# Mrhonor/Mul-Datasets-Semantic-Segmentation

Measured on NVIDIA B200. Metric: labelled pixels/sec (head+OHEM fwd+bwd, mIoU hist), higher is better.
Workload: dtype f32

## Files before the change

mul-datasets-semantic-segmentation_b200/csrc/mds_bwd.cu:

```cuda
#include "tma_util.cuh"

namespace mdseg {
namespace {

using namespace tma;

constexpr int kKC = 8;
constexpr int kBoxW = 36;
constexpr int kStages = 2;
constexpr int kStageFloats = kKC * 2 * kBoxW;
constexpr int kStageBytes = kStageFloats * 4;
constexpr int kCG = 16;
constexpr int kOwn28 = 28;
constexpr int kOwn = kOwn28;
constexpr int kStgW28 = 160;
constexpr int kMaxR = 5;
constexpr int kEnt = 384;
constexpr uint32_t kNoEnt = 0xffffffffu;
#ifndef MDSEG_BWD_BCAST_PIPE
#define MDSEG_BWD_BCAST_PIPE 1
#endif
#ifndef MDSEG_BWD_XP_NOLD
#define MDSEG_BWD_XP_NOLD 0
#endif
#ifndef MDSEG_BWD_XP_NOUSE
#define MDSEG_BWD_XP_NOUSE 0
#endif
#ifndef MDSEG_BWD_XP_NO5
#define MDSEG_BWD_XP_NO5 0
#endif
#ifndef MDSEG_BWD_CHUNK_LEAN
#define MDSEG_BWD_CHUNK_LEAN 1
#endif

template <bool ROW>
struct Lay {
  static constexpr int kOwn = ROW ? 32 : kOwn28;
  static constexpr int kStgW = ROW ? 176 : kStgW28;
  static constexpr size_t kOffCarry = (size_t)kStages * kStageBytes;
  static constexpr size_t kOffLw = kOffCarry + (size_t)kCG * 32 * 4;
  static constexpr size_t kOffLab = kOffLw + (size_t)kMaxR * kStgW * 4;
  static constexpr size_t kOffEnt = kOffLab + (size_t)kMaxR * kStgW;
  static constexpr size_t kOffTile = kOffEnt + (size_t)kEnt * 4;
  static constexpr size_t kOffEptr = kOffTile + (size_t)kKC * kOwn * 4;
  static constexpr size_t kOffBars = kOffEptr + 16;
  static constexpr size_t kOffXbar = kOffBars + (kStages + 1) * 8;
  static constexpr size_t kOffXchg = kOffXbar + 4 * 8;
  static constexpr size_t kOffC5 = (kOffXchg + 2 * kKC * 2 * 4 + 15) / 16 * 16;
  static constexpr size_t kSmem = ROW ? ((kOffC5 + (size_t)kStages * kKC * 8 + 127) / 128) * 128 : kOffXbar;
  static_assert(kCG / kKC + 1 <= 4, "eptr holds one quad offset per chunk of a class group, plus the end");
  static_assert(kOffLw % 16 == 0 && kOffLab % 16 == 0 && kOffEnt % 16 == 0 && kOffTile % 16 == 0 && kOffBars % 8 == 0 &&
                    kOffC5 % 16 == 0,
                "shared memory carve-up alignment");
};
static_assert(Lay<false>::kSmem <= 13568, "16 resident one-warp CTAs per SM need <= 13568 bytes of shared memory each");
static_assert(16 * Lay<true>::kSmem <= 232448, "a 16-warp row CTA must fit the 227 KB of one SM");
constexpr size_t kSmem = Lay<false>::kSmem;
constexpr int kMaxRowWarps = 16;

struct GraphDev {
  const int* csr_ptr;
  const int* csr_col;
  const float* csr_val;
  const int* csc_ptr;
  const int* csr4_ptr;
  const int* csr4_col;
};

struct Args {
  mdseg_src_table src;
  const int32_t* dataset_ids;
  const void* labels;
  Geom gm;
  int ignore;
  const float* loss_px;
  const float* lse_px;
  const mdseg_ohem_state* states;
  const float* grad_out;
  float grad_scale;
  void* out_base[MDSEG_MAX_DATASETS];
  long long out_image_stride[MDSEG_MAX_DATASETS];
  int out_channels[MDSEG_MAX_DATASETS];
  GraphDev g[MDSEG_MAX_DATASETS];
  int zero_invalid;
  float* scrA;
  float* scrB;
  uint8_t* sel8;
  unsigned lite_mask;
  unsigned char lite_strip[kMaxRowWarps];
  int n_lite;
  int c5s;
  float2* col5;
  int c_scr;
  int seg_rows, n_seg, n_strips;
};

__device__ __forceinline__ void bulk_g2s(void* dst, const void* src, uint32_t bytes, uint64_t* bar) {
  asm volatile("cp.async.bulk.shared::cluster.global.mbarrier::complete_tx::bytes [%0], [%1], %2, [%3];" ::"r"(
                   smem_u32(dst)),
               "l"(src), "r"(bytes), "r"(smem_u32(bar))
               : "memory");
}

__device__ __forceinline__ void sts2_if(uint32_t on, uint32_t addr, float a, float b) {
  asm volatile("{ .reg .pred q;\n  setp.ne.u32 q, %0, 0;\n  @q st.shared.v2.f32 [%1], {%2, %3}; }"
               :: "r"(on), "r"(addr), "f"(a), "f"(b) : "memory");
}

__device__ __forceinline__ void sub_onehot2(float2& e, uint32_t lab2, uint32_t c2, float nwabs) {
  asm("{ .reg .pred p, q;\n"
      "  setp.eq.f16x2 p|q, %2, %3;\n"
      "  @p add.f32 %0, %0, %4;\n"
      "  @q add.f32 %1, %1, %4; }"
      : "+f"(e.x), "+f"(e.y)
      : "r"(lab2), "r"(c2), "f"(nwabs));
}

template <typename L>
__global__ void __launch_bounds__(256) mds_bwd_prep_kernel(const Args a, int64_t px_per_image) {
  const int b = blockIdx.y;
  const int d = a.dataset_ids ? a.dataset_ids[b] : 0;
  const bool valid_ds = d >= 0 && d < a.src.n_datasets;
  const int C = valid_ds ? a.src.C[d] : 0;
  SelParams sp;
  sp.thresh = 0.f; sp.kth = 0.f; sp.mode = 0; sp.w = 0.f;
  if (valid_ds) {
    const mdseg_ohem_state* st = a.states + (a.src.seg_per_dataset ? d : 0);
    sp.thresh = st->thresh; sp.kth = st->kth; sp.mode = st->mode;
    sp.w = (a.grad_out ? a.grad_out[a.src.seg_per_dataset ? d : 0] : 1.f) * a.grad_scale * st->inv_n_sel;
  }
  const bool any = valid_ds && fabsf(sp.w) > 0.f;
  const L* labels = (const L*)a.labels;
  const bool lab16 = ((uintptr_t)a.labels & 15) == 0;
  const int64_t base = (int64_t)b * px_per_image;
  for (int64_t q = (int64_t)blockIdx.x * blockDim.x + threadIdx.x; q < px_per_image / 16;
       q += (int64_t)gridDim.x * blockDim.x) {
    const int64_t p = base + q * 16;
    float4 ls[4];
#pragma unroll
    for (int v = 0; v < 4; ++v) ls[v] = __ldcs(reinterpret_cast<const float4*>(a.loss_px + p) + v);
    uint32_t lab[16];
    if (sizeof(L) == 1 && lab16) {
      const uint4 lv = *reinterpret_cast<const uint4*>((const uint8_t*)a.labels + p);
      const uint32_t wv[4] = {lv.x, lv.y, lv.z, lv.w};
#pragma unroll
      for (int i = 0; i < 16; ++i) lab[i] = (wv[i >> 2] >> (8 * (i & 3))) & 0xffu;
    } else {
#pragma unroll
      for (int i = 0; i < 16; ++i) lab[i] = (uint32_t)load_label<L>(labels, p + i);
    }
    uint32_t out[4];
#pragma unroll
    for (int v = 0; v < 4; ++v) {
      const float lsv[4] = {ls[v].x, ls[v].y, ls[v].z, ls[v].w};
      uint32_t packed = 0;
#pragma unroll
// ... 52 lines not shown
#pragma unroll
    for (int i = 0; i < 4; ++i) v[i] = *reinterpret_cast<const float4*>(tile + ((e[i] >> 16) & 7u) * OWN + 4 * t);
#pragma unroll
    for (int i = 0; i < 4; ++i)
      if (col_ok && e[i] != kNoEnt) store4(base + (int64_t)((e[i] & 0xffffu) * (uint32_t)hw), v[i]);
  }
  for (; q < q1; ++q) {
    const uint32_t e = ents[4 * q + o];
    if (col_ok && e != kNoEnt) {
      const float4 v = *reinterpret_cast<const float4*>(tile + (e >> 16) * OWN + 4 * t);
      store4(base + (int64_t)((e & 0xffffu) * (uint32_t)hw), v);
    }
  }
#else
#pragma unroll 4
  for (int q = q0; q < q1; ++q) {
    const uint32_t e = ents[4 * q + o];
    if (col_ok && e != kNoEnt) {
      const float4 v = *reinterpret_cast<const float4*>(tile + (e >> 16) * OWN + 4 * t);
      store4(base + (int64_t)((e & 0xffffu) * (uint32_t)hw), v);
    }
  }
#endif
  __syncwarp();
}

template <typename TO>
__device__ __forceinline__ void store_class(const Args& a, const GraphDev& gd, const Unit& un, TO* outb, int cg, int row,
                                            float v) {
  const int w = a.gm.w;
  if (gd.csr_ptr == nullptr) {
    if (un.own) outb[((int64_t)(un.c_beg + cg) * a.gm.h + row) * w + un.x] = from_f32<TO>(v);
    return;
  }
  const int e0 = __ldg(gd.csr_ptr + un.c_beg + cg), e1 = __ldg(gd.csr_ptr + un.c_beg + cg + 1);
  for (int e = e0; e < e1; ++e) {
    const int u = __ldg(gd.csr_col + e);
    const float val = gd.csr_val ? __ldg(gd.csr_val + e) : 1.f;
    if (un.own) outb[((int64_t)u * a.gm.h + row) * w + un.x] = from_f32<TO>(v * val);
  }
}

template <int STGW>
__device__ __forceinline__ void issue_staging(const Args& a, const Unit& un, int Ys, int R, float* lw2s, uint8_t* labs,
                                              uint64_t* sbar) {
  mbar_expect_tx(sbar, (uint32_t)(R * un.wst * 5));
  for (int j = 0; j < R; ++j) {
    const int64_t p = ((int64_t)un.b * a.gm.H + (Ys + j)) * a.gm.W + un.Xa;
    bulk_g2s(lw2s + j * STGW, a.lse_px + p, (uint32_t)(un.wst * 4), sbar);
    bulk_g2s(labs + j * STGW, a.sel8 + p, (uint32_t)un.wst, sbar);
  }
}

template <bool ROW>
__device__ __noinline__ void skip_chunk(int lane, int k, int cc, bool own, float* scr_first, int64_t scr_stride,
                                        float* carry, float* tile, float* xslot) {
  constexpr int kOwn = Lay<ROW>::kOwn;
  for (int c = 0; c < cc; ++c) {
    if (ROW && xslot != nullptr && lane == 31) { xslot[2 * c] = 0.f; xslot[2 * c + 1] = 0.f; }
    float* cq = carry + (k * kKC + c) * 32 + lane;
    const float rowv = *cq;
    *cq = 0.f;
    if (scr_first != nullptr) {
      if (own) scr_first[c * scr_stride] = 0.f;
    } else if (ROW) {
      tile[c * kOwn + lane] = rowv;
    } else if (lane >= 1 && lane <= kOwn) {
      tile[c * kOwn + lane - 1] = rowv;
    }
  }
}

template <typename TO, int RT, bool NX5, bool ROW>
__device__ __forceinline__ void cell_row(const Args& a, const CUtensorMap* map, const GraphDev& gd, const Unit& un,
                                         TO* outb, int g, int R, int Ys_next, int R_next, const float (&l1w)[5],
                                         const float (&l1h)[kMaxR],
                                         float* stages, uint64_t* bars, float* carry, float* lw2s,
                                         uint8_t* labs, const uint32_t* ents, const int* eptr, float* tile,
                                         float* xmine, uint64_t* xbar_mine, const float* xleft, uint64_t* xbar_left,
                                         bool lite, const float2* c5sm) {
  constexpr int kOwn = Lay<ROW>::kOwn, kStgW = Lay<ROW>::kStgW;
  const int lane = un.lane;
  const float kInf = __int_as_float(0x7f800000);
  float2 LW[RT][2];
  float lw4[RT];
  uint32_t LH[RT][2], lh4[RT];
  uint32_t anysel = 0;
#pragma unroll
  for (int j = 0; j < RT; ++j) {
    float t[5];
    uint32_t hv[5];
#pragma unroll
    for (int i = 0; i < 5; ++i) {
      t[i] = -kInf;
      hv[i] = 255u;
      if (j < R && i < un.nx) {
        hv[i] = labs[j * kStgW + un.sx + i];
        const float off2 = fmaf(-lw2s[j * kStgW + un.sx + i], kLog2e, un.log2w);
        t[i] = hv[i] != 255u ? off2 : -kInf;
      }
      hv[i] = (uint32_t)__half_as_ushort(__ushort2half_rn((unsigned short)hv[i]));
    }
    LW[j][0] = make_float2(t[0], t[1]);
    LW[j][1] = make_float2(t[2], t[3]);
    lw4[j] = t[4];
    LH[j][0] = hv[0] | (hv[1] << 16);
    LH[j][1] = hv[2] | (hv[3] << 16);
    lh4[j] = hv[4] | (0x5bf8u << 16);
    anysel |= (LH[j][0] ^ 0x5bf85bf8u) | (LH[j][1] ^ 0x5bf85bf8u) | (lh4[j] ^ 0x5bf85bf8u);
  }
  __syncwarp();
  if (lane == 0 && g + 1 < un.g1) issue_staging<kStgW>(a, un, Ys_next, R_next, lw2s, labs, &bars[kStages]);
  const bool skip = (ROW || un.cached) && !__any_sync(0xffffffffu, anysel != 0);

  float2 L1H[RT];
#pragma unroll
  for (int j = 0; j < RT; ++j) L1H[j] = dup2(l1h[j]);
  const float2 L1W[2] = {make_float2(l1w[0], l1w[1]), make_float2(l1w[2], l1w[3])};
  const float l1w4 = l1w[4];
  const bool first_partial = (g == un.g0) && (un.g0 > 0);
  TO* orow = outb + (int64_t)g * a.gm.w + un.x0;
  const float nwabs = -fabsf(un.w_signed);
  const float2 K2 = dup2(kLog2e);

#pragma unroll 1
  for (int k = 0; k < un.n_ch; ++k) {
    const int q = (g - un.g0) * un.n_ch + k;
    const int slot = q % kStages;
    const int c_lo = un.c_beg + k * kKC;
    const int cc = (un.c_end - c_lo) < kKC ? (un.c_end - c_lo) : kKC;

    mbar_wait(&bars[slot], (uint32_t)((q / kStages) & 1));
    const int xs = q & 1;
    if (ROW && xmine != nullptr && q >= 2) mbar_wait(&xbar_mine[2 + xs], (uint32_t)(((q >> 1) - 1) & 1));
    const float* Sp = stages + slot * kStageFloats + un.xl;
    if (skip) {
      skip_chunk<ROW>(lane, k, cc, un.own,
                      first_partial ? a.scrA + (((int64_t)un.b * a.n_seg + un.seg) * a.c_scr + c_lo) * a.gm.w + un.x
                                    : nullptr,
                      a.gm.w, carry, tile, xmine ? xmine + xs * kKC * 2 : nullptr);
    } else {
    float n00 = Sp[0], n01 = Sp[1], n10 = Sp[kBoxW], n11 = Sp[kBoxW + 1];
    uint32_t c2 = class_pair(c_lo);
    float* cp = carry + k * kKC * 32 + lane;
    float* tp = tile + (ROW ? lane : lane - 1);
    uint32_t xaddr = 0, xprod = 0;
    if (ROW && xmine != nullptr && lane == 31) { xaddr = smem_u32(xmine + xs * kKC * 2); xprod = 1; }
    asm volatile("" : "+r"(xaddr), "+r"(xprod));
    const float2* x5p = c5sm + slot * kKC;
#pragma unroll 1
    for (int c = 0; c < cc; ++c, c2 = next_class2(c2)) {
      float v00 = n00, v01 = n01, v10 = n10, v11 = n11;
      Sp += 2 * kBoxW;
      if (c + 1 < cc) { n00 = Sp[0]; n01 = Sp[1]; n10 = Sp[kBoxW]; n11 = Sp[kBoxW + 1]; }
      float2 x5 = make_float2(0.f, 0.f);
      if (!NX5 && un.has5 && !MDSEG_BWD_XP_NOLD && !MDSEG_BWD_XP_NOUSE) x5 = x5p[c];
      const float dv0 = v01 - v00, dv1 = v11 - v10;
      const float2 V0 = dup2(v00), DV0 = dup2(dv0), V1 = dup2(v10), DV1 = dup2(dv1);
      float2 CU2, UR2, CL2, LR2;
#pragma unroll
      for (int p = 0; p < 2; ++p) {
        const float2 h0 = fma2(L1W[p], DV0, V0);
        const float2 dd = sub2(fma2(L1W[p], DV1, V1), h0);
        float2 t0, t1;
#pragma unroll
        for (int j = 0; j < RT; ++j) {
          float2 e = ex2_2(fma2(fma2(L1H[j], dd, h0), K2, LW[j][p]));
          sub_onehot2(e, LH[j][p], c2, nwabs);
          t0 = j == 0 ? e : add2(t0, e);
          t1 = j == 0 ? mul2(L1H[j], e) : fma2(L1H[j], e, t1);
        }
        const float2 cu = sub2(t0, t1);
        CU2 = p == 0 ? cu : add2(CU2, cu);
        UR2 = p == 0 ? mul2(L1W[p], cu) : fma2(L1W[p], cu, UR2);
        CL2 = p == 0 ? t1 : add2(CL2, t1);
        LR2 = p == 0 ? mul2(L1W[p], t1) : fma2(L1W[p], t1, LR2);
      }
      float CU = CU2.x + CU2.y, ur = UR2.x + UR2.y, CL = CL2.x + CL2.y, lr = LR2.x + LR2.y;
      if (!NX5 && lite) {
        CU += x5.x; ur = fmaf(l1w4, x5.x, ur);
        CL += x5.y; lr = fmaf(l1w4, x5.y, lr);
      }
      if (NX5) {
        const float h0 = fmaf(l1w4, dv0, v00);
        const float dd = fmaf(l1w4, dv1, v10) - h0;
        float t0 = 0.f, t1 = 0.f;
#pragma unroll
        for (int j = 0; j < RT; ++j) {
          float2 e = make_float2(ex2_approx(fmaf(fmaf(l1h[j], dd, h0), kLog2e, lw4[j])), 0.f);
          sub_onehot2(e, lh4[j], c2, nwabs);
          t0 += e.x;
          t1 = fmaf(l1h[j], e.x, t1);
        }
        const float cu = t0 - t1;
        CU += cu; ur = fmaf(l1w4, cu, ur);
        CL += t1; lr = fmaf(l1w4, t1, lr);
      }
      const float uo = (CU - ur) * un.wsign;
      const float lo = (CL - lr) * un.wsign;
      ur *= un.wsign;
      lr *= un.wsign;
      float gu = __shfl_up_sync(0xffffffffu, ur, 1);
      float gl = __shfl_up_sync(0xffffffffu, lr, 1);
      if (lane == 0) { gu = 0.f; gl = 0.f; }
      if (ROW) {
        sts2_if(xprod, xaddr, ur, lr);
        xaddr += 8;
      }
      const int cg = k * kKC + c;
      const float up = uo + gu;
      const float rowv = up + *cp;
      *cp = lo + gl;
      cp += 32;
      if (first_partial) {
        if (un.own) a.scrA[(((int64_t)un.b * a.n_seg + un.seg) * a.c_scr + (c_lo + c)) * a.gm.w + un.x] = up;
      } else if (ROW || un.cached) {
        if (ROW || (lane >= 1 && lane <= kOwn)) *tp = rowv;
      } else {
        store_class<TO>(a, gd, un, outb, cg, g, rowv);
      }
      tp += kOwn;
    }
    }
    if (ROW) {
      if (xmine != nullptr && lane == 31) mbar_arrive(&xbar_mine[xs]);
      if (xleft != nullptr) {
        mbar_wait(&xbar_left[xs], (uint32_t)((q >> 1) & 1));
        __syncwarp();
        if (lane < cc) {
          const float xu = xleft[(xs * kKC + lane) * 2], xl = xleft[(xs * kKC + lane) * 2 + 1];
          if (first_partial) {
            a.scrA[(((int64_t)un.b * a.n_seg + un.seg) * a.c_scr + (c_lo + lane)) * a.gm.w + un.x0] += xu;
          } else {
            tile[lane * kOwn] += xu;
          }
          carry[(k * kKC + lane) * 32] += xl;
        }
        __syncwarp();
        if (lane == 0) mbar_arrive(&xbar_left[2 + xs]);
      }
    }
    __syncwarp();
    if (lane == 0 && q + kStages < un.n_loads) {
      const int qn = q + kStages;
#if MDSEG_BWD_CHUNK_LEAN
      const int qrow = un.n_ch == 2 ? qn >> 1 : qn, qk = un.n_ch == 2 ? qn & 1 : 0;
#else
      const int qrow = qn / un.n_ch, qk = qn % un.n_ch;
#endif
      mbar_expect_tx(&bars[slot], kStageBytes + (un.c5base ? kKC * 8 : 0));
      load_4d(stages + slot * kStageFloats, map, &bars[slot], un.box_x, un.g0 + qrow, un.c_beg + qk * kKC, un.b);
      if (un.c5base)
        bulk_g2s(const_cast<float2*>(c5sm) + slot * kKC, un.c5base + (un.g0 + qrow) * un.c5row + qk * kKC, kKC * 8,
                 &bars[slot]);
    }
    if (un.cached && !first_partial) broadcast_chunk<TO, kOwn>(un, orow, ents, eptr[k], eptr[k + 1], tile, a.gm.h * a.gm.w);
  }
}

template <typename TO, bool ROW>
__global__ void __launch_bounds__(ROW ? 32 * kMaxRowWarps : 32, ROW ? 1 : 16)
mds_bwd_kernel(const __grid_constant__ Maps maps, const __grid_constant__ Args a) {
  using L = Lay<ROW>;
  constexpr int kOwn = L::kOwn, kStgW = L::kStgW;
  extern __shared__ __align__(128) unsigned char smem_all[];
  const int wi = ROW ? (int)(threadIdx.x >> 5) : 0;
  const int n_w = ROW ? (int)(blockDim.x >> 5) : 1;
  unsigned char* smem_raw = smem_all + (size_t)wi * L::kSmem;
  float* stages = reinterpret_cast<float*>(smem_raw);
  float* carry = reinterpret_cast<float*>(smem_raw + L::kOffCarry);
  float* lw2s = reinterpret_cast<float*>(smem_raw + L::kOffLw);
  uint8_t* labs = smem_raw + L::kOffLab;
  uint32_t* ents = reinterpret_cast<uint32_t*>(smem_raw + L::kOffEnt);
  float* tile = reinterpret_cast<float*>(smem_raw + L::kOffTile);
  int* eptr = reinterpret_cast<int*>(smem_raw + L::kOffEptr);
  uint64_t* bars = reinterpret_cast<uint64_t*>(smem_raw + L::kOffBars);
  float2* c5sm = reinterpret_cast<float2*>(smem_raw + (ROW ? L::kOffC5 : 0));
  const bool has_right = ROW && wi + 1 < n_w, has_left = ROW && wi > 0;
  uint64_t* xbar_mine = has_right ? reinterpret_cast<uint64_t*>(smem_raw + L::kOffXbar) : nullptr;
  float* xmine = has_right ? reinterpret_cast<float*>(smem_raw + L::kOffXchg) : nullptr;
  uint64_t* xbar_left = has_left ? reinterpret_cast<uint64_t*>(smem_raw - L::kSmem + L::kOffXbar) : nullptr;
  const float* xleft = has_left ? reinterpret_cast<const float*>(smem_raw - L::kSmem + L::kOffXchg) : nullptr;

  const Geom& gm = a.gm;
  const int lane = threadIdx.x & 31;
  const int b = blockIdx.z, grp = blockIdx.y;
  const int strip = ROW ? wi : (int)(blockIdx.x % a.n_strips), seg = ROW ? (int)blockIdx.x : (int)(blockIdx.x / a.n_strips);
  const int d = a.dataset_ids ? a.dataset_ids[b] : 0;
  const int h = gm.h, w = gm.w;
  const int x0 = strip * kOwn;
  const int x = ROW ? x0 + lane : x0 + lane - 1;
  const bool own = ROW ? x <= w - 1 : (lane >= 1 && lane <= kOwn && x <= w - 1);
  const int g0 = seg * a.seg_rows;
  const int g1 = (g0 + a.seg_rows < h - 1) ? g0 + a.seg_rows : h - 1;
  const bool last_seg = (g1 == h - 1);

  if (d < 0 || d >= a.src.n_datasets) {
    if (a.zero_invalid && grp == 0) {
      TO* outb = (TO*)a.out_base[0] + (int64_t)b * a.out_image_stride[0];
      for (int u = 0; u < a.out_channels[0]; ++u) zero_rows<TO>(a, outb, u, g0, g1, last_seg, x, own);
    }
    return;
  }
  const int C = a.src.C[d];
  const int c_beg = grp * kCG;
  if (c_beg >= C) return;
  const int c_end = (c_beg + kCG < C) ? c_beg + kCG : C;
  const GraphDev gd = a.g[d];
  TO* outb = (TO*)a.out_base[d] + (int64_t)b * a.out_image_stride[d];
  const mdseg_ohem_state* st = a.states + (a.src.seg_per_dataset ? d : 0);
  const CUtensorMap* map = &maps.m[d];
  const float wsel = (a.grad_out ? a.grad_out[a.src.seg_per_dataset ? d : 0] : 1.f) * a.grad_scale * st->inv_n_sel;

  const bool cell_ok = (x >= 0) && (x <= w - 2) && (ROW || lane <= kOwn);
  int Xbeg = 0, Xend = 0;
  if (cell_ok) cell_span(gm.xm, x, gm.W, Xbeg, Xend);
  const int nx = Xend - Xbeg;
  const unsigned cmask = __ballot_sync(0xffffffffu, cell_ok);
  int Xw0 = 0;
  if (cmask) Xw0 = __shfl_sync(0xffffffffu, Xbeg, __ffs(cmask) - 1);
  float l1w[5];
#pragma unroll
  for (int i = 0; i < 5; ++i) {
    int cell;
    l1w[i] = 0.f;
    if (i < nx) axis_cell(gm.xm, Xbeg + i, cell, l1w[i]);
  }
  const int n5 = __popc(__ballot_sync(0xffffffffu, nx > 4));
  const bool lite = ROW && a.col5 != nullptr && n5 == 1 && ((a.lite_mask >> strip) & 1u);
  const bool nx5 = n5 > 0 && !lite && !MDSEG_BWD_XP_NO5;

  Unit un;
  un.lane = lane; un.b = b; un.seg = seg; un.x = x; un.nx = nx; un.c_beg = c_beg; un.c_end = c_end;
  un.x0 = x0; un.ncols = (w - x0) < kOwn ? (w - x0) : kOwn;
  un.n_ch = (c_end - c_beg + kKC - 1) / kKC;
  un.g0 = g0; un.g1 = g1; un.own = own;
  un.box_x = ROW ? x0 : ((x0 > 0 ? x0 - 1 : 0) & ~3);
  un.xl = cell_ok ? x - un.box_x : 0;
  un.n_loads = (g1 - g0) * un.n_ch;
  un.Xa = Xw0 & ~15;
  un.sx = cell_ok ? Xbeg - un.Xa : 0;
  un.wst = (gm.W - un.Xa) < kStgW ? (gm.W - un.Xa) : kStgW;
  un.w_signed = wsel; un.wsign = wsel < 0.f ? -1.f : 1.f;
  un.log2w = log2f(fabsf(wsel));
  un.cached = false;
  un.has5 = lite && nx > 4 && !MDSEG_BWD_XP_NO5;
  un.c5base = nullptr; un.c5row = 0;
  if (lite && !MDSEG_BWD_XP_NO5 && !MDSEG_BWD_XP_NOLD) {
    un.c5row = (int64_t)(w / 32) * a.c5s;
    un.c5base = a.col5 + ((int64_t)b * (h - 1) * (w / 32) + strip) * a.c5s + c_beg;
  }

  if (lane == 0) {
    prefetch_map(map);
    for (int s = 0; s <= kStages; ++s) mbar_init(&bars[s], 1);
    if (has_right)
      for (int s = 0; s < 4; ++s) mbar_init(&xbar_mine[s], 1);
    mbar_fence_init();
    {
      int Ys0, Ye0;
      cell_span(gm.ym, g0, gm.H, Ys0, Ye0);
      issue_staging<kStgW>(a, un, Ys0, Ye0 - Ys0, lw2s, labs, &bars[kStages]);
    }
    for (int qn = 0; qn < kStages && qn < un.n_loads; ++qn) {
      mbar_expect_tx(&bars[qn], kStageBytes + (un.c5base ? kKC * 8 : 0));
      load_4d(stages + qn * kStageFloats, map, &bars[qn], un.box_x, g0 + qn / un.n_ch, c_beg + (qn % un.n_ch) * kKC,
              b);
      if (un.c5base)
        bulk_g2s(c5sm + qn * kKC, un.c5base + (g0 + qn / un.n_ch) * un.c5row + (qn % un.n_ch) * kKC, kKC * 8, &bars[qn]);
    }
  }
  for (int cg = 0; cg < kCG; ++cg) carry[cg * 32 + lane] = 0.f;
  static_assert(kCG == 2 * kKC, "the channel-list cache is laid out for two chunks per class group");
  if ((gd.csr_ptr == nullptr || gd.csr_val == nullptr) && a.out_channels[d] <= 0xffff &&
      (int64_t)a.out_channels[d] * h * w < 0x7fffffffLL) {
    const int ncls = c_end - c_beg, nc0 = ncls < kKC ? ncls : kKC;
    int myptr = c_beg + lane;
    if (gd.csr_ptr != nullptr) myptr = lane <= ncls ? __ldg(gd.csr_ptr + c_beg + lane) : 0;
    const int p0 = __shfl_sync(0xffffffffu, myptr, 0);
    const int p8 = __shfl_sync(0xffffffffu, myptr, nc0);
    const int pe = __shfl_sync(0xffffffffu, myptr, ncls);
    const int len0 = p8 - p0, len1 = pe - p8;
    const int base1 = (len0 + 3) & ~3;
    const int total = base1 + ((len1 + 3) & ~3);
    if (lane == 0) {
      eptr[0] = 0;
      eptr[1] = base1 >> 2;
      eptr[un.n_ch] = total >> 2;
    }
    for (int eb = 0; eb < pe - p0; eb += 32) {
      const int e = eb + lane;
      int cls = 0;
#pragma unroll
      for (int j = 1; j < kCG; ++j) {
        const int pj = __shfl_sync(0xffffffffu, myptr, j);
        cls += (j < ncls && pj <= p0 + e) ? 1 : 0;
      }
      if (e < pe - p0) {
        const int u = gd.csr_ptr != nullptr ? __ldg(gd.csr_col + p0 + e) : c_beg + e;
        const int pos = cls < kKC ? e : base1 + (e - len0);
        if (pos < kEnt) ents[pos] = (uint32_t)u | ((uint32_t)(cls & (kKC - 1)) << 16);
      }
    }
    if (lane < base1 - len0 && len0 + lane < kEnt) ents[len0 + lane] = kNoEnt;
    if (lane < total - base1 - len1 && base1 + len1 + lane < kEnt) ents[base1 + len1 + lane] = kNoEnt;
    un.cached = total <= kEnt;
  }
  __syncwarp();
  if (ROW) __syncthreads();

  int ys_tab = gm.H;
  if (g0 + lane < h - 1) ys_tab = first_dst_ge(gm.ym, g0 + lane, gm.H);
  for (int g = g0; g < g1; ++g) {
    const int Ys = __shfl_sync(0xffffffffu, ys_tab, g - g0);
    const int Ye = __shfl_sync(0xffffffffu, ys_tab, g - g0 + 1);
    const int R = Ye - Ys;
    float l1h[kMaxR];
#pragma unroll
    for (int j = 0; j < kMaxR; ++j) {
      int cell;
      l1h[j] = 0.f;
      if (j < R) axis_cell(gm.ym, Ys + j, cell, l1h[j]);
    }
    const int Rn = __shfl_sync(0xffffffffu, ys_tab, (g - g0 + 2) & 31) - Ye;
    mbar_wait(&bars[kStages], (uint32_t)((g - g0) & 1));
#define MDSEG_ROW(RT, N5)                                                                                           \
  cell_row<TO, RT, N5, ROW>(a, map, gd, un, outb, g, R, Ye, Rn, l1w, l1h, stages, bars, carry, lw2s, labs, ents, eptr, \
                            tile, xmine, xbar_mine, xleft, xbar_left, lite, c5sm)
    if (R <= 4) {
      if (nx5) MDSEG_ROW(4, true); else MDSEG_ROW(4, false);
    } else {
      if (nx5) MDSEG_ROW(5, true); else MDSEG_ROW(5, false);
    }
#undef MDSEG_ROW
  }

  if (last_seg && un.cached) {
    TO* olast = outb + (int64_t)(h - 1) * w + x0;
    for (int k = 0; k < un.n_ch; ++k) {
      for (int j = 0; j < kKC && k * kKC + j < c_end - c_beg; ++j)
        if (ROW) tile[j * kOwn + lane] = carry[(k * kKC + j) * 32 + lane];
        else if (lane >= 1 && lane <= kOwn) tile[j * kOwn + lane - 1] = carry[(k * kKC + j) * 32 + lane];
      __syncwarp();
      broadcast_chunk<TO, kOwn>(un, olast, ents, eptr[k], eptr[k + 1], tile, h * w);
    }
  } else {
    for (int cg = 0; cg < c_end - c_beg; ++cg) {
      const float v = carry[cg * 32 + lane];
      if (last_seg) {
        store_class<TO>(a, gd, un, outb, cg, h - 1, v);
      } else if (own) {
        a.scrB[(((int64_t)b * a.n_seg + (seg + 1)) * a.c_scr + (c_beg + cg)) * w + x] = v;
      }
    }
  }
  if (grp == 0 && gd.csr_ptr != nullptr && gd.csc_ptr != nullptr) {
    for (int u0 = 0; u0 < a.out_channels[d]; u0 += 32) {
      const int u = u0 + lane;
      const bool empty = u < a.out_channels[d] && __ldg(gd.csc_ptr + u) == __ldg(gd.csc_ptr + u + 1);
      unsigned m = __ballot_sync(0xffffffffu, empty);
      while (m) {
        const int uu = u0 + __ffs(m) - 1;
        m &= m - 1;
        zero_rows<TO>(a, outb, uu, g0, g1, last_seg, x, own);
      }
    }
  }
}

__global__ void __launch_bounds__(32 * kMaxRowWarps) mds_bwd_col5_kernel(const Args a) {
  const Geom& gm = a.gm;
  const int lane = threadIdx.x & 31, strip = a.lite_strip[threadIdx.x >> 5], n_w = a.gm.w / 32;
  const int g = blockIdx.x, b = blockIdx.y;
  const int d = a.dataset_ids ? a.dataset_ids[b] : 0;
  if (d < 0 || d >= a.src.n_datasets) return;
  const int h = gm.h, w = gm.w;
  const int x = strip * 32 + lane;
  int Xbeg = 0, Xend = 0;
  if (x <= w - 2) cell_span(gm.xm, x, gm.W, Xbeg, Xend);
  const unsigned m5 = __ballot_sync(0xffffffffu, Xend - Xbeg > 4);
  if (__popc(m5) != 1) return;
  const int owner = __ffs(m5) - 1;
  const int xo = strip * 32 + owner;
  const int X5 = __shfl_sync(0xffffffffu, Xbeg, owner) + 4;
  int cell;
  float l1w4;
  axis_cell(gm.xm, X5, cell, l1w4);
  int Ys, Ye;
  cell_span(gm.ym, g, gm.H, Ys, Ye);
  const int R = Ye - Ys;
  const int C = a.src.C[d];
  const mdseg_ohem_state* st = a.states + (a.src.seg_per_dataset ? d : 0);
  const float wsel = (a.grad_out ? a.grad_out[a.src.seg_per_dataset ? d : 0] : 1.f) * a.grad_scale * st->inv_n_sel;
  const float log2w = log2f(fabsf(wsel)), nwabs = -fabsf(wsel);
  const float kInf = __int_as_float(0x7f800000);
  float l1h[kMaxR], off[kMaxR];
  int cls[kMaxR];
#pragma unroll
  for (int j = 0; j < kMaxR; ++j) {
    l1h[j] = 0.f; off[j] = -kInf; cls[j] = 255;
    if (j < R) {
      axis_cell(gm.ym, Ys + j, cell, l1h[j]);
      const int64_t p = ((int64_t)b * gm.H + (Ys + j)) * gm.W + X5;
      cls[j] = a.sel8[p];
      if (cls[j] != 255) off[j] = fmaf(-a.lse_px[p], kLog2e, log2w);
    }
  }
  const float* yb = (const float*)a.src.base[d] + (int64_t)b * a.src.image_stride[d] + (int64_t)g * w + xo;
// ... 24 lines not shown
  const int d = a.dataset_ids ? a.dataset_ids[b] : 0;
  if (d < 0 || d >= a.src.n_datasets) return;
  const int C = a.src.C[d];
  const int w = a.gm.w, h = a.gm.h, w4 = w / 4;
  const int idx = blockIdx.x * blockDim.x + threadIdx.x;
  const int cls = idx / w4, x4 = idx - cls * w4;
  if (cls >= C) return;
  const int row = k * a.seg_rows;
  const int64_t so = (((int64_t)b * a.n_seg + k) * a.c_scr + cls) * w + x4 * 4;
  const float4 A = *reinterpret_cast<const float4*>(a.scrA + so);
  const float4 B = *reinterpret_cast<const float4*>(a.scrB + so);
  const float v[4] = {A.x + B.x, A.y + B.y, A.z + B.z, A.w + B.w};
  const GraphDev gd = a.g[d];
  TO* outb = (TO*)a.out_base[d] + (int64_t)b * a.out_image_stride[d];
  if (gd.csr_ptr == nullptr) {
    TO* o = outb + ((int64_t)cls * h + row) * w + x4 * 4;
#pragma unroll
    for (int i = 0; i < 4; ++i) o[i] = from_f32<TO>(v[i]);
    return;
  }
  const int e0 = __ldg(gd.csr_ptr + cls), e1 = __ldg(gd.csr_ptr + cls + 1);
  for (int e = e0; e < e1; ++e) {
    const int u = __ldg(gd.csr_col + e);
    const float val = gd.csr_val ? __ldg(gd.csr_val + e) : 1.f;
    TO* o = outb + ((int64_t)u * h + row) * w + x4 * 4;
#pragma unroll
    for (int i = 0; i < 4; ++i) o[i] = from_f32<TO>(v[i] * val);
  }
}

#ifndef MDSEG_SEG_ROWS
#define MDSEG_SEG_ROWS 16
#endif
int pick_seg_rows(int h, int w, int n_images, int c_max) {
  int sr = h - 1 < MDSEG_SEG_ROWS ? h - 1 : MDSEG_SEG_ROWS;
  if (sr < 1) sr = 1;
  if (!(w % 32 == 0 && w / 32 <= kMaxRowWarps)) return sr;
  const long long per_seg = (long long)n_images * ((c_max + kCG - 1) / kCG);
  while (sr > 4 && per_seg * ((h - 1 + sr - 1) / sr) < sm_count()) sr /= 2;
  return sr;
}

template <typename L>
int launch_prep(const Args& a, int n_images, cudaStream_t s) {
  const int64_t ppi = (int64_t)a.gm.H * a.gm.W;
  int64_t bx = ceil_div64(ppi / 16, 256);
  const int64_t want = ceil_div64((int64_t)sm_count() * 16, n_images);
  if (bx > want) bx = want;
  mds_bwd_prep_kernel<L><<<dim3((unsigned)bx, (unsigned)n_images), 256, 0, s>>>(a, ppi);
  MDSEG_LAUNCH_OK();
  return 0;
}

bool row_route(const Args& a, bool ents_fit) {
  return ents_fit && a.gm.w % 32 == 0 && a.gm.w / 32 <= kMaxRowWarps;
}

template <typename TO>
int launch(int label_dtype, const Maps& maps, const Args& a, int n_images, int max_c, bool ents_fit, cudaStream_t s) {
  int rc = 2;
  switch (label_dtype) {
    case MDSEG_U8: rc = launch_prep<uint8_t>(a, n_images, s); break;
    case MDSEG_I32: rc = launch_prep<int32_t>(a, n_images, s); break;
    case MDSEG_I64: rc = launch_prep<int64_t>(a, n_images, s); break;
    default: set_error("mdseg_mds_bwd: unsupported label dtype %d", label_dtype);
  }
  if (rc) return rc;
  if (row_route(a, ents_fit)) {
    const int n_w = a.gm.w / 32;
    if (a.col5 != nullptr && a.n_lite > 0) {
      mds_bwd_col5_kernel<<<dim3((unsigned)(a.gm.h - 1), (unsigned)n_images), 32 * a.n_lite, 0, s>>>(a);
      MDSEG_LAUNCH_OK();
    }
    const size_t smem = (size_t)n_w * Lay<true>::kSmem;
    auto k = mds_bwd_kernel<TO, true>;
    MDSEG_CUDA_OK(cudaFuncSetAttribute(k, cudaFuncAttributeMaxDynamicSharedMemorySize, (int)smem));
    dim3 grid((unsigned)a.n_seg, (unsigned)((max_c + kCG - 1) / kCG), (unsigned)n_images);
    k<<<grid, 32 * n_w, smem, s>>>(maps, a);
  } else {
    auto k = mds_bwd_kernel<TO, false>;
    MDSEG_CUDA_OK(cudaFuncSetAttribute(k, cudaFuncAttributeMaxDynamicSharedMemorySize, (int)kSmem));
    dim3 grid((unsigned)(a.n_strips * a.n_seg), (unsigned)((max_c + kCG - 1) / kCG), (unsigned)n_images);
    k<<<grid, 32, kSmem, s>>>(maps, a);
  }
  MDSEG_LAUNCH_OK();
  if (a.n_seg > 1) {
    dim3 g2((unsigned)(((int64_t)max_c * (a.gm.w / 4) + 255) / 256), (unsigned)(a.n_seg - 1), (unsigned)n_images);
    mds_bwd_fixup_kernel<TO><<<g2, 256, 0, s>>>(a);
    MDSEG_LAUNCH_OK();
  }
  return 0;
}

size_t col5_bytes(int n_images, int h, int w, int c_max) {
  if (w % 32 != 0 || w / 32 > kMaxRowWarps || h < 2) return 0;
  return (size_t)n_images * (h - 1) * (w / 32) * ((c_max + kKC - 1) / kKC * kKC) * sizeof(float2) + 16;
}

void pick_lite_strips(Args& a) {
  a.lite_mask = 0; a.n_lite = 0;
  if (a.col5 == nullptr) return;
  const int w = a.gm.w, W = a.gm.W;
  int n5[kMaxRowWarps] = {0};
  int cols = 0, cur = 0;
  for (int X = 0; X <= W; ++X) {
    int cell = w - 2;
    if (X < W) {
      const int i0 = (int)(a.gm.xm.scale * (float)X);
      cell = i0 > w - 2 ? w - 2 : i0;
    }
    if (X == W || cell != cur) {
      if (cols > 4 && cur / 32 < kMaxRowWarps) ++n5[cur / 32];
      cur = cell; cols = 0;
    }
    ++cols;
  }
  for (int st = 0; st < w / 32 && st < kMaxRowWarps; ++st)
    if (n5[st] == 1) {
      a.lite_mask |= 1u << st;
      a.lite_strip[a.n_lite++] = (unsigned char)st;
    }
}

int src_max_c(const mdseg_src_table* s) {
  int m = 0;
  for (int i = 0; i < s->n_datasets; ++i) m = s->C[i] > m ? s->C[i] : m;
  return m;
// ... 229 lines not shown
```

Baseline: 11.10 billion.

## Stage full gradient rows in shared memory and write them with bulk async copies

On the row route, each warp now writes its per-chunk gradient tile into a CTA-wide double-buffered row buffer instead of a per-warp tile. The last warp to finish a chunk, found through a shared-memory atomic ticket, broadcasts whole rows to every mapped output channel with cp.async.bulk shared-to-global copies. Mbarriers guard buffer reuse. The aim is to replace many small per-warp scattered global stores with full-row bulk transfers, at the cost of cross-warp synchronisation, serialised issue by a single lane, and a new alignment check on the output.

```diff
diff --git a/mul-datasets-semantic-segmentation_b200/csrc/mds_bwd.cu b/mul-datasets-semantic-segmentation_b200/csrc/mds_bwd.cu
--- a/mul-datasets-semantic-segmentation_b200/csrc/mds_bwd.cu
+++ b/mul-datasets-semantic-segmentation_b200/csrc/mds_bwd.cu
@@ -29,21 +29,28 @@
 #ifndef MDSEG_BWD_XP_NO5
 #define MDSEG_BWD_XP_NO5 0
 #endif
+#ifndef MDSEG_BWD_XP_NOBCAST
+#define MDSEG_BWD_XP_NOBCAST 0
+#endif
 #ifndef MDSEG_BWD_CHUNK_LEAN
 #define MDSEG_BWD_CHUNK_LEAN 1
+#endif
+#ifndef MDSEG_BWD_ROWSTORE
+#define MDSEG_BWD_ROWSTORE 1
 #endif
 
 template <bool ROW>
 struct Lay {
   static constexpr int kOwn = ROW ? 32 : kOwn28;
   static constexpr int kStgW = ROW ? 176 : kStgW28;
+  static constexpr bool kWarpEnts = !(ROW && MDSEG_BWD_ROWSTORE);
   static constexpr size_t kOffCarry = (size_t)kStages * kStageBytes;
   static constexpr size_t kOffLw = kOffCarry + (size_t)kCG * 32 * 4;
   static constexpr size_t kOffLab = kOffLw + (size_t)kMaxR * kStgW * 4;
   static constexpr size_t kOffEnt = kOffLab + (size_t)kMaxR * kStgW;
-  static constexpr size_t kOffTile = kOffEnt + (size_t)kEnt * 4;
-  static constexpr size_t kOffEptr = kOffTile + (size_t)kKC * kOwn * 4;
-  static constexpr size_t kOffBars = kOffEptr + 16;
+  static constexpr size_t kOffTile = kOffEnt + (kWarpEnts ? (size_t)kEnt * 4 : 0);
+  static constexpr size_t kOffEptr = kOffTile + (kWarpEnts ? (size_t)kKC * kOwn * 4 : 0);
+  static constexpr size_t kOffBars = kOffEptr + (kWarpEnts ? 16 : 0);
   static constexpr size_t kOffXbar = kOffBars + (kStages + 1) * 8;
   static constexpr size_t kOffXchg = kOffXbar + 4 * 8;
   static constexpr size_t kOffC5 = (kOffXchg + 2 * kKC * 2 * 4 + 15) / 16 * 16;
@@ -53,10 +60,29 @@
                     kOffC5 % 16 == 0,
                 "shared memory carve-up alignment");
 };
+constexpr int kMaxRowWarps = 16;
+struct RowTail {
+  __host__ __device__ static constexpr size_t kOffEnt(int w) { return (size_t)2 * kKC * w * 4; }
+  __host__ __device__ static constexpr size_t kOffEptr(int w) { return kOffEnt(w) + (size_t)kEnt * 4; }
+  __host__ __device__ static constexpr size_t kOffTicket(int w) { return kOffEptr(w) + 16; }
+  __host__ __device__ static constexpr size_t kOffBars(int w) { return kOffTicket(w) + 2 * 4; }
+  __host__ __device__ static constexpr size_t kBytes(int w) { return kOffBars(w) + 2 * 8; }
+};
+struct RowStore {
+  float* rows;
+  const uint32_t* ents;
+  const int* eptr;
+  unsigned* ticket;
+  uint64_t* empty;
+  int n_w;
+  bool cached;
+};
 static_assert(Lay<false>::kSmem <= 13568, "16 resident one-warp CTAs per SM need <= 13568 bytes of shared memory each");
-static_assert(16 * Lay<true>::kSmem <= 232448, "a 16-warp row CTA must fit the 227 KB of one SM");
+static_assert(kMaxRowWarps * Lay<true>::kSmem + (MDSEG_BWD_ROWSTORE ? RowTail::kBytes(32 * kMaxRowWarps) : 0) <= 232448,
+              "a 16-warp row CTA must fit the 227 KB of one SM");
+static_assert(Lay<true>::kSmem % 16 == 0 && RowTail::kOffBars(32) % 8 == 0, "bulk copies read 16-byte aligned rows");
 constexpr size_t kSmem = Lay<false>::kSmem;
-constexpr int kMaxRowWarps = 16;
+constexpr size_t row_smem(int n_w) { return (size_t)n_w * Lay<true>::kSmem + (MDSEG_BWD_ROWSTORE ? RowTail::kBytes(32 * n_w) : 0); }
 
 struct GraphDev {
   const int* csr_ptr;
@@ -102,6 +128,15 @@
                : "memory");
 }
 
+__device__ __forceinline__ void bulk_s2g(void* dst, const void* src, uint32_t bytes) {
+  asm volatile("cp.async.bulk.global.shared::cta.bulk_group [%0], [%1], %2;" ::"l"(dst), "r"(smem_u32(src)), "r"(bytes)
+               : "memory");
+}
+__device__ __forceinline__ void bulk_commit() { asm volatile("cp.async.bulk.commit_group;" ::: "memory"); }
+__device__ __forceinline__ void bulk_wait_read() { asm volatile("cp.async.bulk.wait_group.read 0;" ::: "memory"); }
+__device__ __forceinline__ void bulk_wait_all() { asm volatile("cp.async.bulk.wait_group 0;" ::: "memory"); }
+__device__ __forceinline__ void fence_async_smem() { asm volatile("fence.proxy.async.shared::cta;" ::: "memory"); }
+
 __device__ __forceinline__ void sts2_if(uint32_t on, uint32_t addr, float a, float b) {
   asm volatile("{ .reg .pred q;\n  setp.ne.u32 q, %0, 0;\n  @q st.shared.v2.f32 [%1], {%2, %3}; }"
                :: "r"(on), "r"(addr), "f"(a), "f"(b) : "memory");
@@ -260,10 +295,63 @@
   }
 }
 
+template <typename TO>
+__device__ __noinline__ void rows_out(const Args& a, const RowStore& rs, TO* outb, int lane, int s, int row, int k,
+                                      int cc) {
+  const int h = a.gm.h, w = a.gm.w;
+  float* buf = rs.rows + s * kKC * w;
+  if (rs.cached) {
+    if constexpr (sizeof(TO) == 2) {
+      __syncwarp();
+      for (int c = 0; c < cc; ++c) {
+        const float2* src = reinterpret_cast<const float2*>(buf + c * w);
+        TO* dst = reinterpret_cast<TO*>(buf) + c * w;
+        float2 v[kMaxRowWarps / 2];
+#pragma unroll
+        for (int i = 0; i < kMaxRowWarps / 2; ++i)
+          if (lane + 32 * i < w / 2) v[i] = src[lane + 32 * i];
+        __syncwarp();
+#pragma unroll
+        for (int i = 0; i < kMaxRowWarps / 2; ++i)
+          if (lane + 32 * i < w / 2) {
+            dst[2 * (lane + 32 * i)] = from_f32<TO>(v[i].x);
+            dst[2 * (lane + 32 * i) + 1] = from_f32<TO>(v[i].y);
+          }
+        __syncwarp();
+      }
+      fence_async_smem();
+      __syncwarp();
+    }
+    if (lane == 0) {
+      const unsigned char* src = reinterpret_cast<const unsigned char*>(buf);
+      const uint32_t bytes = (uint32_t)(w * sizeof(TO));
+      for (int i = 4 * rs.eptr[k]; i < 4 * rs.eptr[k + 1]; ++i) {
+        const uint32_t e = rs.ents[i];
+        if (e != kNoEnt) bulk_s2g(outb + ((int64_t)(e & 0xffffu) * h + row) * w, src + ((e >> 16) & 7u) * bytes, bytes);
+      }
+      bulk_commit();
+      bulk_wait_read();
+    }
+  }
+  if (lane == 0) mbar_arrive(&rs.empty[s]);
+  __syncwarp();
+}
+
+template <typename TO>
+__device__ __forceinline__ void rows_done(const Args& a, const RowStore& rs, TO* outb, int lane, int s, int row, int k,
+                                          int cc) {
+  fence_async_smem();
+  __syncwarp();
+  unsigned t = 0;
+  if (lane == 0)
+    asm volatile("atom.acq_rel.cta.shared::cta.inc.u32 %0, [%1], %2;"
+                 : "=r"(t) : "r"(smem_u32(&rs.ticket[s])), "r"((unsigned)rs.n_w - 1) : "memory");
+  if (__shfl_sync(0xffffffffu, t, 0) == (unsigned)rs.n_w - 1) rows_out<TO>(a, rs, outb, lane, s, row, k, cc);
+}
+
 template <bool ROW>
 __device__ __noinline__ void skip_chunk(int lane, int k, int cc, bool own, float* scr_first, int64_t scr_stride,
-                                        float* carry, float* tile, float* xslot) {
-  constexpr int kOwn = Lay<ROW>::kOwn;
+                                        float* carry, float* tile, int ts, float* xslot) {
   for (int c = 0; c < cc; ++c) {
     if (ROW && xslot != nullptr && lane == 31) { xslot[2 * c] = 0.f; xslot[2 * c + 1] = 0.f; }
     float* cq = carry + (k * kKC + c) * 32 + lane;
@@ -272,9 +360,9 @@
     if (scr_first != nullptr) {
       if (own) scr_first[c * scr_stride] = 0.f;
     } else if (ROW) {
-      tile[c * kOwn + lane] = rowv;
-    } else if (lane >= 1 && lane <= kOwn) {
-      tile[c * kOwn + lane - 1] = rowv;
+      tile[c * ts + lane] = rowv;
+    } else if (lane >= 1 && lane <= Lay<ROW>::kOwn) {
+      tile[c * ts + lane - 1] = rowv;
     }
   }
 }
@@ -286,8 +374,10 @@
                                          float* stages, uint64_t* bars, float* carry, float* lw2s,
                                          uint8_t* labs, const uint32_t* ents, const int* eptr, float* tile,
                                          float* xmine, uint64_t* xbar_mine, const float* xleft, uint64_t* xbar_left,
-                                         bool lite, const float2* c5sm) {
+                                         bool lite, const float2* c5sm, const RowStore& rs) {
   constexpr int kOwn = Lay<ROW>::kOwn, kStgW = Lay<ROW>::kStgW;
+  constexpr bool kRS = ROW && MDSEG_BWD_ROWSTORE;
+  const int ts = kRS ? a.gm.w : kOwn;
   const int lane = un.lane;
   const float kInf = __int_as_float(0x7f800000);
   float2 LW[RT][2];
@@ -341,17 +431,20 @@
     mbar_wait(&bars[slot], (uint32_t)((q / kStages) & 1));
     const int xs = q & 1;
     if (ROW && xmine != nullptr && q >= 2) mbar_wait(&xbar_mine[2 + xs], (uint32_t)(((q >> 1) - 1) & 1));
+    const int qb = q - (un.g0 > 0 ? un.n_ch : 0);
+    float* tl = kRS ? rs.rows + (qb & 1) * kKC * a.gm.w + un.x0 : tile;
+    if (kRS && !first_partial && qb >= 2) mbar_wait(&rs.empty[qb & 1], (uint32_t)(((qb >> 1) - 1) & 1));
     const float* Sp = stages + slot * kStageFloats + un.xl;
     if (skip) {
       skip_chunk<ROW>(lane, k, cc, un.own,
                       first_partial ? a.scrA + (((int64_t)un.b * a.n_seg + un.seg) * a.c_scr + c_lo) * a.gm.w + un.x
                                     : nullptr,
-                      a.gm.w, carry, tile, xmine ? xmine + xs * kKC * 2 : nullptr);
+                      a.gm.w, carry, tl, ts, xmine ? xmine + xs * kKC * 2 : nullptr);
     } else {
     float n00 = Sp[0], n01 = Sp[1], n10 = Sp[kBoxW], n11 = Sp[kBoxW + 1];
     uint32_t c2 = class_pair(c_lo);
     float* cp = carry + k * kKC * 32 + lane;
-    float* tp = tile + (ROW ? lane : lane - 1);
+    float* tp = tl + (ROW ? lane : lane - 1);
     uint32_t xaddr = 0, xprod = 0;
     if (ROW && xmine != nullptr && lane == 31) { xaddr = smem_u32(xmine + xs * kKC * 2); xprod = 1; }
     asm volatile("" : "+r"(xaddr), "+r"(xprod));
@@ -427,7 +520,7 @@
       } else {
         store_class<TO>(a, gd, un, outb, cg, g, rowv);
       }
-      tp += kOwn;
+      tp += ts;
     }
     }
     if (ROW) {
@@ -440,7 +533,7 @@
           if (first_partial) {
             a.scrA[(((int64_t)un.b * a.n_seg + un.seg) * a.c_scr + (c_lo + lane)) * a.gm.w + un.x0] += xu;
           } else {
-            tile[lane * kOwn] += xu;
+            tl[lane * ts] += xu;
           }
           carry[(k * kKC + lane) * 32] += xl;
         }
@@ -462,8 +555,51 @@
         bulk_g2s(const_cast<float2*>(c5sm) + slot * kKC, un.c5base + (un.g0 + qrow) * un.c5row + qk * kKC, kKC * 8,
                  &bars[slot]);
     }
-    if (un.cached && !first_partial) broadcast_chunk<TO, kOwn>(un, orow, ents, eptr[k], eptr[k + 1], tile, a.gm.h * a.gm.w);
-  }
+    if (kRS) {
+      if (!first_partial) rows_done<TO>(a, rs, outb, lane, qb & 1, g, k, cc);
+    } else if (un.cached && !first_partial && !MDSEG_BWD_XP_NOBCAST) {
+      broadcast_chunk<TO, kOwn>(un, orow, ents, eptr[k], eptr[k + 1], tile, a.gm.h * a.gm.w);
+    }
+  }
+}
+
+__device__ __forceinline__ bool build_ents(const Args& a, const GraphDev& gd, int d, int c_beg, int c_end, int n_ch,
+                                           int lane, uint32_t* ents, int* eptr) {
+  static_assert(kCG == 2 * kKC, "the channel-list cache is laid out for two chunks per class group");
+  if (!((gd.csr_ptr == nullptr || gd.csr_val == nullptr) && a.out_channels[d] <= 0xffff &&
+        (int64_t)a.out_channels[d] * a.gm.h * a.gm.w < 0x7fffffffLL))
+    return false;
+  const int ncls = c_end - c_beg, nc0 = ncls < kKC ? ncls : kKC;
+  int myptr = c_beg + lane;
+  if (gd.csr_ptr != nullptr) myptr = lane <= ncls ? __ldg(gd.csr_ptr + c_beg + lane) : 0;
+  const int p0 = __shfl_sync(0xffffffffu, myptr, 0);
+  const int p8 = __shfl_sync(0xffffffffu, myptr, nc0);
+  const int pe = __shfl_sync(0xffffffffu, myptr, ncls);
+  const int len0 = p8 - p0, len1 = pe - p8;
+  const int base1 = (len0 + 3) & ~3;
+  const int total = base1 + ((len1 + 3) & ~3);
+  if (lane == 0) {
+    eptr[0] = 0;
+    eptr[1] = base1 >> 2;
+    eptr[n_ch] = total >> 2;
+  }
+  for (int eb = 0; eb < pe - p0; eb += 32) {
+    const int e = eb + lane;
+    int cls = 0;
+#pragma unroll
+    for (int j = 1; j < kCG; ++j) {
+      const int pj = __shfl_sync(0xffffffffu, myptr, j);
+      cls += (j < ncls && pj <= p0 + e) ? 1 : 0;
+    }
+    if (e < pe - p0) {
+      const int u = gd.csr_ptr != nullptr ? __ldg(gd.csr_col + p0 + e) : c_beg + e;
+      const int pos = cls < kKC ? e : base1 + (e - len0);
+      if (pos < kEnt) ents[pos] = (uint32_t)u | ((uint32_t)(cls & (kKC - 1)) << 16);
+    }
+  }
+  if (lane < base1 - len0 && len0 + lane < kEnt) ents[len0 + lane] = kNoEnt;
+  if (lane < total - base1 - len1 && base1 + len1 + lane < kEnt) ents[base1 + len1 + lane] = kNoEnt;
+  return total <= kEnt;
 }
 
 template <typename TO, bool ROW>
@@ -471,17 +607,21 @@
 mds_bwd_kernel(const __grid_constant__ Maps maps, const __grid_constant__ Args a) {
   using L = Lay<ROW>;
   constexpr int kOwn = L::kOwn, kStgW = L::kStgW;
+  constexpr bool kRS = ROW && MDSEG_BWD_ROWSTORE;
   extern __shared__ __align__(128) unsigned char smem_all[];
   const int wi = ROW ? (int)(threadIdx.x >> 5) : 0;
   const int n_w = ROW ? (int)(blockDim.x >> 5) : 1;
   unsigned char* smem_raw = smem_all + (size_t)wi * L::kSmem;
+  unsigned char* tail = smem_all + (size_t)n_w * L::kSmem;
   float* stages = reinterpret_cast<float*>(smem_raw);
   float* carry = reinterpret_cast<float*>(smem_raw + L::kOffCarry);
   float* lw2s = reinterpret_cast<float*>(smem_raw + L::kOffLw);
   uint8_t* labs = smem_raw + L::kOffLab;
-  uint32_t* ents = reinterpret_cast<uint32_t*>(smem_raw + L::kOffEnt);
+  uint32_t* ents = reinterpret_cast<uint32_t*>(kRS ? tail + RowTail::kOffEnt(32 * n_w) : smem_raw + L::kOffEnt);
   float* tile = reinterpret_cast<float*>(smem_raw + L::kOffTile);
-  int* eptr = reinterpret_cast<int*>(smem_raw + L::kOffEptr);
+  int* eptr = reinterpret_cast<int*>(kRS ? tail + RowTail::kOffEptr(32 * n_w) : smem_raw + L::kOffEptr);
+  RowStore rs{reinterpret_cast<float*>(tail), ents, eptr, reinterpret_cast<unsigned*>(tail + RowTail::kOffTicket(32 * n_w)),
+              reinterpret_cast<uint64_t*>(tail + RowTail::kOffBars(32 * n_w)), n_w, false};
   uint64_t* bars = reinterpret_cast<uint64_t*>(smem_raw + L::kOffBars);
   float2* c5sm = reinterpret_cast<float2*>(smem_raw + (ROW ? L::kOffC5 : 0));
   const bool has_right = ROW && wi + 1 < n_w, has_left = ROW && wi > 0;
@@ -579,43 +719,25 @@
     }
   }
   for (int cg = 0; cg < kCG; ++cg) carry[cg * 32 + lane] = 0.f;
-  static_assert(kCG == 2 * kKC, "the channel-list cache is laid out for two chunks per class group");
-  if ((gd.csr_ptr == nullptr || gd.csr_val == nullptr) && a.out_channels[d] <= 0xffff &&
-      (int64_t)a.out_channels[d] * h * w < 0x7fffffffLL) {
-    const int ncls = c_end - c_beg, nc0 = ncls < kKC ? ncls : kKC;
-    int myptr = c_beg + lane;
-    if (gd.csr_ptr != nullptr) myptr = lane <= ncls ? __ldg(gd.csr_ptr + c_beg + lane) : 0;
-    const int p0 = __shfl_sync(0xffffffffu, myptr, 0);
-    const int p8 = __shfl_sync(0xffffffffu, myptr, nc0);
-    const int pe = __shfl_sync(0xffffffffu, myptr, ncls);
-    const int len0 = p8 - p0, len1 = pe - p8;
-    const int base1 = (len0 + 3) & ~3;
-    const int total = base1 + ((len1 + 3) & ~3);
-    if (lane == 0) {
-      eptr[0] = 0;
-      eptr[1] = base1 >> 2;
-      eptr[un.n_ch] = total >> 2;
-    }
-    for (int eb = 0; eb < pe - p0; eb += 32) {
-      const int e = eb + lane;
-      int cls = 0;
-#pragma unroll
-      for (int j = 1; j < kCG; ++j) {
-        const int pj = __shfl_sync(0xffffffffu, myptr, j);
-        cls += (j < ncls && pj <= p0 + e) ? 1 : 0;
-      }
-      if (e < pe - p0) {
-        const int u = gd.csr_ptr != nullptr ? __ldg(gd.csr_col + p0 + e) : c_beg + e;
-        const int pos = cls < kKC ? e : base1 + (e - len0);
-        if (pos < kEnt) ents[pos] = (uint32_t)u | ((uint32_t)(cls & (kKC - 1)) << 16);
-      }
-    }
-    if (lane < base1 - len0 && len0 + lane < kEnt) ents[len0 + lane] = kNoEnt;
-    if (lane < total - base1 - len1 && base1 + len1 + lane < kEnt) ents[base1 + len1 + lane] = kNoEnt;
-    un.cached = total <= kEnt;
-  }
-  __syncwarp();
-  if (ROW) __syncthreads();
+  if (kRS) {
+    if (wi == 0) {
+      const bool cached = build_ents(a, gd, d, c_beg, c_end, un.n_ch, lane, ents, eptr);
+      if (lane == 0) {
+        eptr[3] = cached ? 1 : 0;
+        rs.ticket[0] = 0;
+        rs.ticket[1] = 0;
+        for (int s = 0; s < 2; ++s) mbar_init(&rs.empty[s], 1);
+        mbar_fence_init();
+      }
+    }
+    __syncthreads();
+    un.cached = eptr[3] != 0;
+    rs.cached = un.cached;
+  } else {
+    un.cached = build_ents(a, gd, d, c_beg, c_end, un.n_ch, lane, ents, eptr);
+    __syncwarp();
+    if (ROW) __syncthreads();
+  }
 
   int ys_tab = gm.H;
   if (g0 + lane < h - 1) ys_tab = first_dst_ge(gm.ym, g0 + lane, gm.H);
@@ -634,7 +756,7 @@
     mbar_wait(&bars[kStages], (uint32_t)((g - g0) & 1));
 #define MDSEG_ROW(RT, N5)                                                                                           \
   cell_row<TO, RT, N5, ROW>(a, map, gd, un, outb, g, R, Ye, Rn, l1w, l1h, stages, bars, carry, lw2s, labs, ents, eptr, \
-                            tile, xmine, xbar_mine, xleft, xbar_left, lite, c5sm)
+                            tile, xmine, xbar_mine, xleft, xbar_left, lite, c5sm, rs)
     if (R <= 4) {
       if (nx5) MDSEG_ROW(4, true); else MDSEG_ROW(4, false);
     } else {
@@ -643,7 +765,17 @@
 #undef MDSEG_ROW
   }
 
-  if (last_seg && un.cached) {
+  if (kRS && last_seg && un.cached) {
+    const int qb0 = (g1 - g0 - (g0 > 0 ? 1 : 0)) * un.n_ch;
+    for (int k = 0; k < un.n_ch; ++k) {
+      const int qb = qb0 + k;
+      float* tl = rs.rows + (qb & 1) * kKC * w + x0;
+      if (qb >= 2) mbar_wait(&rs.empty[qb & 1], (uint32_t)(((qb >> 1) - 1) & 1));
+      const int cc = (c_end - c_beg - k * kKC) < kKC ? (c_end - c_beg - k * kKC) : kKC;
+      for (int j = 0; j < cc; ++j) tl[j * w + lane] = carry[(k * kKC + j) * 32 + lane];
+      rows_done<TO>(a, rs, outb, lane, qb & 1, h - 1, k, cc);
+    }
+  } else if (last_seg && un.cached) {
     TO* olast = outb + (int64_t)(h - 1) * w + x0;
     for (int k = 0; k < un.n_ch; ++k) {
       for (int j = 0; j < kKC && k * kKC + j < c_end - c_beg; ++j)
@@ -662,6 +794,7 @@
       }
     }
   }
+  if (kRS && lane == 0) bulk_wait_all();
   if (grp == 0 && gd.csr_ptr != nullptr && gd.csc_ptr != nullptr) {
     for (int u0 = 0; u0 < a.out_channels[d]; u0 += 32) {
       const int u = u0 + lane;
@@ -792,8 +925,11 @@
   return 0;
 }
 
-bool row_route(const Args& a, bool ents_fit) {
-  return ents_fit && a.gm.w % 32 == 0 && a.gm.w / 32 <= kMaxRowWarps;
+bool row_route(const Args& a, bool ents_fit, size_t out_size) {
+  bool aligned = true;
+  for (int i = 0; i < a.src.n_datasets; ++i)
+    aligned = aligned && ((uintptr_t)a.out_base[i] & 15) == 0 && (a.out_image_stride[i] * (long long)out_size) % 16 == 0;
+  return ents_fit && a.gm.w % 32 == 0 && a.gm.w / 32 <= kMaxRowWarps && (aligned || !MDSEG_BWD_ROWSTORE);
 }
 
 template <typename TO>
@@ -806,13 +942,13 @@
     default: set_error("mdseg_mds_bwd: unsupported label dtype %d", label_dtype);
   }
   if (rc) return rc;
-  if (row_route(a, ents_fit)) {
+  if (row_route(a, ents_fit, sizeof(TO))) {
     const int n_w = a.gm.w / 32;
     if (a.col5 != nullptr && a.n_lite > 0) {
       mds_bwd_col5_kernel<<<dim3((unsigned)(a.gm.h - 1), (unsigned)n_images), 32 * a.n_lite, 0, s>>>(a);
       MDSEG_LAUNCH_OK();
     }
-    const size_t smem = (size_t)n_w * Lay<true>::kSmem;
+    const size_t smem = row_smem(n_w);
     auto k = mds_bwd_kernel<TO, true>;
     MDSEG_CUDA_OK(cudaFuncSetAttribute(k, cudaFuncAttributeMaxDynamicSharedMemorySize, (int)smem));
     dim3 grid((unsigned)a.n_seg, (unsigned)((max_c + kCG - 1) / kCG), (unsigned)n_images);
diff --git a/profiles/rowstore_fullgrad.py b/profiles/rowstore_fullgrad.py
--- /dev/null
+++ b/profiles/rowstore_fullgrad.py
@@ -0,0 +1,37 @@
+import hashlib
+import json
+import os
+import sys
+
+import numpy as np
+import torch
+
+ROOT = os.path.dirname(os.path.dirname(os.path.abspath(__file__)))
+sys.path.insert(0, ROOT)
+import bench
+from mdseg_b200 import ops
+
+DT = {"f32": torch.float32, "bf16": torch.bfloat16, "f16": torch.float16}
+
+
+def fingerprint(workload, logits, dtype):
+    dev = torch.device("cuda:0")
+    bt = bench.make_batch(workload, dev, 1234, logits=logits)
+    graphs = [g.to(dev) for g in bt["graphs"]]
+    luts = torch.from_numpy(np.stack(bt["luts"])).to(dev)
+    ids_t = torch.tensor(bt["ids"], dtype=torch.int32, device=dev)
+    labels = ops.lut_remap_images(bt["raw"], luts, ids_t, out_dtype=torch.int64)
+    x = bt["x"].to(DT[dtype]).requires_grad_(True)
+    loss = ops.mds_proj_ohem_ce(x, labels, ids_t, graphs, ops.neg_log(0.4))
+    loss.backward()
+    torch.cuda.synchronize()
+    ops.check_errors(dev)
+    g = x.grad.contiguous().view(torch.uint8).cpu().numpy()
+    return {"case": f"{workload}:{logits}:{dtype}", "loss": float(loss), "numel": x.grad.numel(),
+            "sha256": hashlib.sha256(g.tobytes()).hexdigest()}
+
+
+if __name__ == "__main__":
+    cases = sys.argv[1:] or ["cfg3:randn:f32", "cfg3:mixed:f32", "cfg3:randn:bf16"]
+    for c in cases:
+        print(json.dumps(fingerprint(*c.split(":"))), flush=True)
```

Measured after the change: 8.067 billion, median of 6. 27.3% lower.
